# DanbiAubrey/Hypergraph_diffusion_for_recommendation

Hardware: AMD Instinct MI355X
Metric: hypergraph-conv fwd+bwd M-edges/sec at emb_dim=64; % HBM roofline (higher is better)
Workload: dtype f32

## Files before the change

hypergraph_diffusion_for_recommendation_amd/_native.py:

```python
from __future__ import annotations

import ctypes
import os
import threading

_HERE = os.path.dirname(os.path.abspath(__file__))
LIB_PATH = os.environ.get("HGD_LIB_PATH", os.path.join(_HERE, "_lib", "libhgd.so"))

c_void_p = ctypes.c_void_p
c_i64 = ctypes.c_int64
c_i32 = ctypes.c_int32
c_f32 = ctypes.c_float
c_f64 = ctypes.c_double
c_size = ctypes.c_size_t

HGD_OK = 0
EPI_NONE, EPI_LEAKY_RELU, EPI_RELU = 0, 1, 2
DT_F32, DT_BF16 = 0, 1
_STATUS_NAMES = {0: "HGD_OK", 1: "HGD_ERR_INVALID_ARG", 2: "HGD_ERR_HIP",
                 3: "HGD_ERR_UNSUPPORTED", 4: "HGD_ERR_WORKSPACE"}


class HGDNativeError(RuntimeError):
    """Raised when libhgd is missing or a call returns a non-OK hgd_status."""
# ... 195 lines not shown
                                   c_i64, c_i64, c_i64, c_void_p, c_i32, c_i64, c_void_p, c_i32,
                                   c_i64, c_i32, c_i32, c_f32, ctypes.POINTER(SplitPlan),
                                   c_void_p, c_size, c_void_p]),
    "hgd_spmm_blocks_for": (c_i32, [c_i64, c_i32]),
    "hgd_spmm_col_blocks_workspace_size": (c_size, [c_i64, c_i32]),
    "hgd_spmm_col_blocks": (c_i32, [c_void_p, c_void_p, c_i64, c_i64, c_i32, c_void_p, c_void_p,
                                    c_void_p, c_void_p, c_size, c_void_p]),
    "hgd_spmm_blocked": (c_i32, [c_void_p, c_void_p, c_void_p, c_void_p, c_i64, c_i64, c_i64,
                                 c_i64, c_void_p, c_i64, c_void_p, c_i64, c_i32, c_i32, c_f32,
                                 c_i32, c_void_p]),
    "hgd_spmm_blocked_dt_workspace_size": (c_size, [c_i64, c_i32, c_i32, c_i32]),
    "hgd_spmm_blocked_dt": (c_i32, [c_void_p, c_void_p, c_void_p, c_void_p, c_i64, c_i64, c_i64,
                                    c_i64, c_void_p, c_i32, c_i64, c_void_p, c_i32, c_i64, c_i32,
                                    c_i32, c_f32, c_i32, c_void_p, c_size, c_void_p]),
    "hgd_spmm_blocks_for_dt": (c_i32, [c_i64, c_i32, c_i32]),
    "hgd_spmm_row_order_for": (c_i32, [c_i64, c_i64, c_i64, c_i32]),
    "hgd_spmm_row_order_workspace_size": (c_size, [c_i64]),
    "hgd_spmm_row_order": (c_i32, [c_void_p, c_void_p, c_i64, c_i64, c_void_p, c_void_p,
                                   c_void_p, c_void_p, c_void_p, c_size, c_void_p]),
    "hgd_spmm_ordered": (c_i32, [c_void_p, c_void_p, c_void_p, c_void_p, c_i64, c_i64, c_i64,
                                 c_i64, c_void_p, c_i64, c_void_p, c_i64, c_i32, c_i32, c_f32,
                                 ctypes.POINTER(SplitPlan), c_void_p, c_size, c_void_p,
                                 c_void_p]),
    "hgd_spmm_masked": (c_i32, [c_void_p, c_void_p, c_void_p, c_void_p, c_f32, c_void_p, c_i64,
                                c_i64, c_i64, c_i64, c_void_p, c_i64, c_void_p, c_i64, c_i32,
                                c_i32, c_f32, ctypes.POINTER(SplitPlan), c_void_p, c_size,
                                c_void_p]),
    "hgd_spmm_masked_fused": (c_i32, [c_void_p, c_void_p, c_void_p, c_void_p, c_f32, c_void_p,
                                      c_i64, c_i64, c_i64, c_i64, c_void_p, c_i64, c_void_p,
                                      c_i64, c_i32, ctypes.POINTER(RowEpilogue),
                                      ctypes.POINTER(SplitPlan), c_void_p, c_size, c_void_p]),
    "hgd_spmm_fused": (c_i32, [c_void_p, c_void_p, c_void_p, c_void_p, c_i64, c_i64, c_i64,
                               c_i64, c_void_p, c_i64, c_void_p, c_i64, c_i32,
                               ctypes.POINTER(RowEpilogue), ctypes.POINTER(SplitPlan), c_void_p,
                               c_size, c_void_p]),
    "hgd_row_epilogue_forward": (c_i32, [c_void_p, c_i64, c_i64, c_i32,
                                         ctypes.POINTER(RowEpilogue), c_void_p, c_i64,
                                         c_void_p]),
    "hgd_row_epilogue_backward_workspace_size": (c_size, [c_i64, c_i32]),
    "hgd_row_epilogue_backward": (c_i32, [c_void_p, c_i64, c_void_p, c_i64, c_void_p, c_void_p,
                                          c_i64, c_i32, c_i32, c_f32, c_i32, c_f32, c_void_p,
                                          c_i64, c_void_p, c_void_p, c_void_p, c_size,
                                          c_void_p]),
    "hgd_linear_forward": (c_i32, [c_void_p, c_i64, c_i64, c_i32, c_void_p, c_i64, c_i32,
                                   c_void_p, c_i32, c_void_p, c_i64, c_void_p]),
    "hgd_linear_backward_data": (c_i32, [c_void_p, c_i64, c_void_p, c_i64, c_i64, c_i32,
# ... 319 lines not shown
```

hypergraph_diffusion_for_recommendation_amd/csrc/spmm.hip:

```cpp
#include <cmath>

#include <hipcub/hipcub.hpp>

#include "spmm_launch.h"

extern "C" size_t hgd_spmm_workspace_size(const hgd_split_plan* plan, int32_t d) {
  if (!plan || plan->n_heavy <= 0 || plan->threshold <= 0 || d <= 0) return 0;
  return hgd::align_up(static_cast<size_t>(plan->n_chunks) * static_cast<size_t>(d) * 4);
}

namespace hgd {
namespace {

__device__ __forceinline__ int32_t advance_block(int64_t c, int32_t k, int64_t n_cols,
                                                 int32_t n_blk) {
  while (k + 1 < n_blk && c >= n_cols * (k + 1) / n_blk) ++k;
  return k;
}

__global__ void col_block_count_kernel(const int64_t* __restrict__ rowptr,
                                       const int32_t* __restrict__ col, int64_t n_rows,
                                       int64_t n_cols, int32_t n_blk, int64_t* __restrict__ cnt) {
  const int64_t r = static_cast<int64_t>(blockIdx.x) * blockDim.x + threadIdx.x;
  if (r == 0) cnt[static_cast<int64_t>(n_blk) * n_rows] = 0;
// ... 80 lines not shown
  for (int64_t i = l; i < n; i += kOrdG) {
    col_o[dst + i] = col[src + i];
    perm[dst + i] = static_cast<int32_t>(src + i);
  }
}

struct RowOrderWs {
  size_t keys, keys_s, len, tail, total;
};

RowOrderWs row_order_ws(int64_t n_rows) {
  RowOrderWs w{};
  size_t scan = 0;
  if (hipcub::DeviceScan::ExclusiveSum(nullptr, scan, static_cast<const int64_t*>(nullptr),
                                       static_cast<int64_t*>(nullptr), n_rows + 1) != hipSuccess)
    return w;
  const size_t sort = hgd_sort_perm_workspace_size(n_rows);
  if (sort == 0) return w;
  const size_t k = align_up(static_cast<size_t>(n_rows) * sizeof(int32_t));
  w.keys = 0;
  w.keys_s = k;
  w.len = 2 * k;
  w.tail = w.len + align_up(static_cast<size_t>(n_rows + 1) * sizeof(int64_t));
  w.total = w.tail + (sort > align_up(scan) ? sort : align_up(scan));
  return w;
}

}
}

extern "C" size_t hgd_spmm_row_order_workspace_size(int64_t n_rows) {
  if (n_rows <= 0 || n_rows >= 0x7fffffffLL) return 0;
  return hgd::row_order_ws(n_rows).total;
}

extern "C" hgd_status hgd_spmm_row_order(const int64_t* rowptr, const int32_t* col,
                                         int64_t n_rows, int64_t n_cols, int32_t* order,
                                         int64_t* rowptr_o, int32_t* col_o, int32_t* perm,
                                         void* workspace, size_t workspace_bytes, void* stream) {
  using namespace hgd;
  clear_error();
  HGD_REQUIRE(n_rows >= 0 && n_cols >= 0, "hgd_spmm_row_order: negative sizes");
  HGD_REQUIRE(n_rows < 0x7fffffffLL, "hgd_spmm_row_order: n_rows >= 2^31 - 1");
  HGD_REQUIRE(n_cols < 0x7fffffffLL, "hgd_spmm_row_order: n_cols >= 2^31 - 1");
  if (n_rows == 0) return HGD_OK;
  HGD_REQUIRE(rowptr && order && rowptr_o, "hgd_spmm_row_order: null rowptr / order / rowptr_o");
// ... 16 lines not shown
  s = hgd_sort_perm(keys, n_rows, n_cols + 1, keys_s, order, ws + w.tail, workspace_bytes - w.tail,
                    stream);
  if (s != HGD_OK) return s;
  hipLaunchKernelGGL(row_order_len_kernel, dim3(grid_for(n_rows + 1)), dim3(kBlock), 0, st, rowptr,
                     order, n_rows, len);
  s = check_launch("hgd_spmm_row_order lengths");
  if (s != HGD_OK) return s;
  size_t tail_bytes = workspace_bytes - w.tail;
  HGD_HIP(hipcub::DeviceScan::ExclusiveSum(ws + w.tail, tail_bytes, len, rowptr_o, n_rows + 1, st));
  hipLaunchKernelGGL(row_order_copy_kernel, dim3(grid), dim3(kBlock), 0, st, rowptr, col, order,
                     rowptr_o, n_rows, col_o, perm);
  return check_launch("hgd_spmm_row_order copy");
}

extern "C" int32_t hgd_spmm_row_order_for(int64_t n_rows, int64_t n_src_rows, int64_t nnz,
                                          int32_t d) {
  if (n_rows <= 0 || n_src_rows <= 0 || nnz <= 0 || d <= 0) return 0;
  const double table = static_cast<double>(n_src_rows) * (d <= 128 ? d : 64) * 4.0;
  if (table < 33554432.0) return 0;
  if (nnz > 32 * n_rows) return 0;
  return 1;
}

extern "C" hgd_status hgd_spmm_ordered(const int64_t* rowptr, const int32_t* col,
                                       const float* val, const float* row_scale, int64_t n_rows,
                                       int64_t n_src_rows, int64_t row_begin, int64_t row_end,
                                       const float* X, int64_t ldx, float* Y, int64_t ldy,
                                       int32_t d, int32_t epilogue, float slope,
                                       const hgd_split_plan* plan, void* workspace,
                                       size_t workspace_bytes, const int32_t* out_row,
                                       void* stream) {
  hgd::clear_error();
  hgd::SpmmRequest r{"hgd_spmm_ordered", rowptr, col, val, row_scale, n_rows, n_src_rows, row_begin,
                     row_end, X, ldx, Y, ldy, d, epilogue, slope, plan, workspace, workspace_bytes,
                     stream};
  r.ordered = true;
  r.out_row = out_row;
  return hgd::spmm_launch<float, float>(r);
}

extern "C" hgd_status hgd_spmm(const int64_t* rowptr, const int32_t* col, const float* val,
                               const float* row_scale, int64_t n_rows, int64_t n_src_rows,
                               int64_t row_begin, int64_t row_end, const float* X, int64_t ldx,
                               float* Y, int64_t ldy, int32_t d, int32_t epilogue, float slope,
                               const hgd_split_plan* plan, void* workspace,
                               size_t workspace_bytes, void* stream) {
// ... 54 lines not shown
  if (s != HGD_OK) return s;
  HGD_HIP(hipcub::DeviceScan::ExclusiveSum(tmp, tmp_bytes, cnt, blk_start, n, st));
  hipLaunchKernelGGL(col_block_scatter_kernel, dim3(grid), dim3(256), 0, st, rowptr, col, n_rows,
                     n_cols, n_blocks, blk_start, blk_col, blk_perm);
  return check_launch("hgd_spmm_col_blocks scatter");
}

extern "C" hgd_status hgd_spmm_blocked(const int64_t* blk_start, const int32_t* blk_col,
                                       const float* blk_val, const float* row_scale,
                                       int64_t n_rows, int64_t n_src_rows, int64_t row_begin,
                                       int64_t row_end, const float* X, int64_t ldx, float* Y,
                                       int64_t ldy, int32_t d, int32_t epilogue, float slope,
                                       int32_t n_blocks, void* stream) {
  hgd::clear_error();
  hgd::SpmmRequest r{"hgd_spmm_blocked", nullptr, blk_col, blk_val, row_scale, n_rows, n_src_rows,
                     row_begin, row_end, X, ldx, Y, ldy, d, epilogue, slope};
  r.blocked = true;
  r.blk_start = blk_start;
  r.n_blk = n_blocks;
  r.stream = stream;
  return hgd::spmm_launch<float, float>(r);
}

extern "C" hgd_status hgd_spmm_fused(const int64_t* rowptr, const int32_t* col, const float* val,
                                     const float* row_scale, int64_t n_rows, int64_t n_src_rows,
                                     int64_t row_begin, int64_t row_end, const float* X,
                                     int64_t ldx, float* Y, int64_t ldy, int32_t d,
                                     const hgd_row_epilogue* epi, const hgd_split_plan* plan,
                                     void* workspace, size_t workspace_bytes, void* stream) {
  hgd::clear_error();
  HGD_REQUIRE(epi != nullptr, "hgd_spmm_fused: null epilogue descriptor");
  hgd::SpmmRequest r{"hgd_spmm_fused", rowptr, col, val, row_scale, n_rows, n_src_rows, row_begin,
                     row_end, X, ldx, Y, ldy, d, epi->act, epi->slope, plan, workspace,
                     workspace_bytes, stream};
  r.ex = epi;
  return hgd::spmm_launch<float, float>(r);
}

extern "C" hgd_status hgd_spmm_masked(const int64_t* rowptr, const int32_t* col, const float* val,
                                      const uint8_t* mask, float keep, const float* row_scale,
                                      int64_t n_rows, int64_t n_src_rows, int64_t row_begin,
                                      int64_t row_end, const float* X, int64_t ldx, float* Y,
                                      int64_t ldy, int32_t d, int32_t epilogue, float slope,
                                      const hgd_split_plan* plan, void* workspace,
                                      size_t workspace_bytes, void* stream) {
  hgd::clear_error();
// ... 30 lines not shown
```

hypergraph_diffusion_for_recommendation_amd/csrc/spmm_launch.h:

```cpp
#pragma once

#include <cmath>
#include <type_traits>

#include "spmm_kernels.h"

namespace hgd {

constexpr int kDefaultPolicy = kPolPrefetch;
static_assert(SpmmTuning{}.policy == kDefaultPolicy && SpmmTuning{}.unroll == 8);

template <class TX, class TY>
constexpr bool kF32 = std::is_same_v<TX, float> && std::is_same_v<TY, float>;

struct SpmmRequest {
  const char* fn;
  const int64_t* rowptr;
  const int32_t* col;
  const float* val;
  const float* row_scale;
  int64_t n_rows, n_src_rows;
  int64_t row_begin, row_end;
  const void* X;
  int64_t ldx;
// ... 109 lines not shown
    case 16: return launch_g<16, VEC, EX>(a, r);
    case 32: return launch_g<32, VEC, EX>(a, r);
    case 64:
      if constexpr (VEC != 8) return launch_g<64, VEC, EX>(a, r);
      [[fallthrough]];
    default: return fail(HGD_ERR_UNSUPPORTED, "%s: unsupported group size %d", r.fn, G);
  }
}

inline size_t blocked_part_bytes(int64_t n_rows, int32_t d, size_t sy, int32_t n_blk) {
  if (sy != 2 || n_blk <= 1 || n_rows <= 0 || d <= 0) return 0;
  return align_up(static_cast<size_t>(n_rows) * static_cast<size_t>(d) * 4);
}

inline bool has_split_rows(const hgd_split_plan* plan) {
  return plan && plan->threshold > 0 && plan->n_heavy > 0;
}

inline hgd_status spmm_check_args(const SpmmRequest& r) {
  const char* fn = r.fn;
  const int32_t d = r.d;
  const hgd_row_epilogue* ex = r.ex;
  const bool empty = r.row_end == r.row_begin;
  HGD_REQUIRE(!r.ordered || r.out_row || r.n_rows <= 0, "%s: null out_row", fn);
  HGD_REQUIRE(!r.blocked || (r.n_blk >= 1 && r.n_blk <= 64), "%s: blocks must be 1..64", fn);
  HGD_REQUIRE(!r.blocked || r.blk_start || r.row_end <= r.row_begin, "%s: null blk_start", fn);
  HGD_REQUIRE(r.keep > 0.f, "%s: keep must be > 0 (got %g)", fn, (double)r.keep);
  HGD_REQUIRE(!r.masked || r.mask || empty, "%s: null mask", fn);
  HGD_REQUIRE(d > 0, "%s: d must be > 0 (got %d)", fn, d);
  HGD_REQUIRE(r.n_rows >= 0 && r.n_src_rows >= 0, "%s: negative sizes", fn);
  HGD_REQUIRE(r.row_begin >= 0 && r.row_begin <= r.row_end && r.row_end <= r.n_rows,
              "%s: row range [%lld,%lld) outside [0,%lld)", fn, (long long)r.row_begin,
              (long long)r.row_end, (long long)r.n_rows);
  HGD_REQUIRE(r.ldx >= d && r.ldy >= d, "%s: ldx/ldy must be >= d", fn);
  HGD_REQUIRE(r.epilogue >= HGD_EPI_NONE && r.epilogue <= HGD_EPI_RELU, "%s: bad epilogue %d", fn,
              r.epilogue);
  if (ex) {
    HGD_REQUIRE(r.epilogue == HGD_EPI_NONE || r.slope >= 0.f,
                "%s: a fused activation needs slope >= 0 (got %g)", fn, (double)r.slope);
    HGD_REQUIRE(ex->layer_norm == 0 || ex->layer_norm == 1, "%s: layer_norm must be 0/1", fn);
    HGD_REQUIRE(!ex->res1 || ex->ld_res1 >= d, "%s: ld_res1 < d", fn);
    HGD_REQUIRE(!ex->res2 || ex->ld_res2 >= d, "%s: ld_res2 < d", fn);
    HGD_REQUIRE(!ex->act_out || ex->ld_act >= d, "%s: ld_act < d", fn);
    HGD_REQUIRE((ex->sum_out == nullptr) == (ex->sum_res == nullptr),
                "%s: sum_out and sum_res go together", fn);
    HGD_REQUIRE(!ex->sum_out || (ex->ld_sum_out >= d && ex->ld_sum_res >= d),
                "%s: ld_sum_out / ld_sum_res < d", fn);
  }
  if (!empty) {
    HGD_REQUIRE((r.rowptr || r.blocked) && r.Y, "%s: null rowptr/Y", fn);
    HGD_REQUIRE(r.X || r.n_src_rows == 0, "%s: null X", fn);
  }
  if (r.out_row) {
    if (has_split_rows(r.plan) || (r.plan && (r.plan->flags & HGD_PLAN_SEGMENTED)))
      return fail(HGD_ERR_UNSUPPORTED, "%s: no split rows or segmented walk with a row order", fn);
    if (r.mask || ex || r.blocked)
      return fail(HGD_ERR_UNSUPPORTED,
                  "%s: no mask, fused row epilogue or source blocks with a row order", fn);
    if (r.row_begin != 0 || r.row_end != r.n_rows)
      return fail(HGD_ERR_UNSUPPORTED, "%s: a row order covers all rows, got [%lld,%lld) of %lld",
                  fn, (long long)r.row_begin, (long long)r.row_end, (long long)r.n_rows);
  }
  return HGD_OK;
}

template <class TX, class TY>
hgd_status spmm_fill_args(SpmmArgsT<TX, TY>& a, const SpmmRequest& r) {
  const SpmmTuning& t = spmm_tuning();
  a.rowptr = r.rowptr;
  a.col = r.col;
  a.val = r.val;
  a.row_scale = r.row_scale;
  a.row_begin = r.row_begin;
  a.row_end = r.row_end;
  a.X = static_cast<const TX*>(r.X);
  a.ldx = r.ldx;
  a.Y = static_cast<TY*>(r.Y);
  a.ldy = r.ldy;
  a.d = r.d;
  a.epi = r.epilogue;
  a.slope = r.slope;
// ... 85 lines not shown
  return HGD_OK;
}

template <int VEC, class TX, class TY>
hgd_status spmm_passes(SpmmArgsT<TX, TY> a, const SpmmRequest& r, const SpmmPassPlan& p) {
  const int32_t d = a.d;
  const bool fused = r.ex != nullptr;
  if constexpr (kF32<TX, TY> && VEC == 4) {
    const int n_pass = (d + p.step - 1) / p.step;
    if (spmm_tuning().pass_interleave && n_pass > 1 && !fused && !r.blocked && !a.mask &&
        a.n_chunks == 0 && !a.seg) {
      a.col0 = 0;
      a.n_pass = n_pass;
      a.pass_cols = p.step;
      return launch_vec<VEC, false>(p.G, a, r);
    }
  }
  for (int c0 = 0; c0 < d; c0 += p.step) {
    a.col0 = c0;
    for (int k = 0; k < (r.blocked ? r.n_blk : 1); ++k) {
      hgd_status s;
      if (r.blocked) {
        a.rowptr = r.blk_start + static_cast<int64_t>(k) * r.n_rows;
        if constexpr (kF32<TX, TY>) {
          if (VEC == 4) a.seg = spmm_tuning().blocked_seg;
        }
        a.blk_accum = k > 0;
        a.epi = k + 1 == r.n_blk ? r.epilogue : HGD_EPI_NONE;
        a.blk_last = k + 1 == r.n_blk;
      }
      if constexpr (kF32<TX, TY>) {
        s = fused ? launch_vec<VEC, true>(p.G, a, r) : launch_vec<VEC, false>(p.G, a, r);
      } else {
        s = launch_vec<VEC, false>(p.G, a, r);
      }
      if (s != HGD_OK) return s;
    }
  }
  return HGD_OK;
}

template <class TX, class TY>
hgd_status spmm_launch(const SpmmRequest& r) {
  hgd_status s = spmm_check_args(r);
  if (s != HGD_OK || r.row_end == r.row_begin) return s;
  SpmmArgsT<TX, TY> a{};
  s = spmm_fill_args(a, r);
// ... 10 lines not shown
```

hypergraph_diffusion_for_recommendation_amd/incidence.py:

```python
from __future__ import annotations

import copy
import ctypes
import os
import weakref
from typing import Dict, Optional, Tuple

import torch

from . import _native as nat
from . import profiling

DEFAULT_SPLIT_THRESHOLD = 2048
DEFAULT_SPLIT_CHUNK = 512
SPLIT_THRESHOLD_MIN = 128
SPLIT_NNZ_PER_THRESHOLD = 8192
SEGMENTED_MAX_AVG_DEGREE = 32
TARGET_GROUPS = 16384


def auto_split(n_rows: int, nnz: int) -> Tuple[int, int]:
    if n_rows >= TARGET_GROUPS or nnz == 0:
        t = SPLIT_THRESHOLD_MIN
        while 2 * t <= nnz // SPLIT_NNZ_PER_THRESHOLD and t < DEFAULT_SPLIT_THRESHOLD:
# ... 11 lines not shown


def _stream(device) -> int:
    return nat.stream_handle(device)


class CSR:

    def __init__(self, rowptr: torch.Tensor, col: torch.Tensor, n_rows: int, n_cols: int,
                 split_threshold: int = DEFAULT_SPLIT_THRESHOLD,
                 split_chunk: int = DEFAULT_SPLIT_CHUNK, plan_counts: Optional[Tuple] = None):
        self.rowptr = rowptr
        self.col = col
        self._ws_bytes: Dict[int, int] = {}
        self.n_rows = int(n_rows)
        self.n_cols = int(n_cols)
        self.nnz = int(col.numel())
        self.device = rowptr.device
        self.split_threshold = int(split_threshold)
        self.split_chunk = int(split_chunk)
        self.cols_ascending = False
        self._col_blocks: Dict[int, Tuple[torch.Tensor, torch.Tensor, torch.Tensor]] = {}
        self._blk_vals: Dict[Tuple[int, int], tuple] = {}
        self._row_order: Optional[Tuple[torch.Tensor, ...]] = None
        self._ord_vals: Dict[Tuple[int, int], tuple] = {}
        self._plan_arrays = ()
        self.plan = nat.SplitPlan()
        self.plan.threshold = 0
        if plan_counts is not None:
            self._build_plan(*plan_counts)

    def plan_count_async(self) -> Optional[torch.Tensor]:
        if self.split_threshold <= 0 or self.n_rows == 0 or self.nnz <= self.split_threshold:
            return None
        counts = torch.empty(2, dtype=torch.int64, device=self.device)
        nat.check(nat.load().hgd_split_plan_count(
            self.rowptr.data_ptr(), self.n_rows, self.split_threshold, self.split_chunk,
            counts.data_ptr(), _stream(self.device)), "hgd_split_plan_count")
        return counts

    def _build_plan(self, n_heavy: int, n_chunks: int) -> None:
        self._ws_bytes = {}
        n_heavy, n_chunks = int(n_heavy), int(n_chunks)
        if n_heavy == 0:
            self.plan.threshold = 0
            return
# ... 41 lines not shown
                raise RuntimeError("col_blocks: the rows' columns are not known to be ascending")
            dev = self.device
            lib = nat.load()
            start = torch.empty(n_blocks * self.n_rows + 1, dtype=torch.int64, device=dev)
            bcol = torch.empty(self.nnz, dtype=torch.int32, device=dev)
            perm = torch.empty(self.nnz, dtype=torch.int32, device=dev)
            if self.n_rows:
                ws = _ws(lib.hgd_spmm_col_blocks_workspace_size(self.n_rows, n_blocks), dev)
                nat.check(lib.hgd_spmm_col_blocks(
                    self.rowptr.data_ptr(), self.col.data_ptr() if self.nnz else None,
                    self.n_rows, self.n_cols, n_blocks, start.data_ptr(),
                    bcol.data_ptr() if self.nnz else None, perm.data_ptr() if self.nnz else None,
                    ws.data_ptr(), ws.numel(), _stream(dev)), "hgd_spmm_col_blocks")
            else:
                start.zero_()
            got = self._col_blocks[n_blocks] = (start, bcol, perm)
        return got

    def blocked_values(self, n_blocks: int, val: Optional[torch.Tensor]) -> Optional[torch.Tensor]:
        if val is None:
            return None
        return _gather32_cached(self._blk_vals, n_blocks, val, self.col_blocks(n_blocks)[2])

    def row_order(self) -> Tuple[torch.Tensor, torch.Tensor, torch.Tensor, torch.Tensor]:
        got = self._row_order
        if got is None:
            dev = self.device
            lib = nat.load()
            order = torch.empty(self.n_rows, dtype=torch.int32, device=dev)
            rowptr_o = torch.empty(self.n_rows + 1, dtype=torch.int64, device=dev)
            col_o = torch.empty(self.nnz, dtype=torch.int32, device=dev)
            perm = torch.empty(self.nnz, dtype=torch.int32, device=dev)
            if self.n_rows:
                ws = _ws(lib.hgd_spmm_row_order_workspace_size(self.n_rows), dev)
                nat.check(lib.hgd_spmm_row_order(
                    self.rowptr.data_ptr(), self.col.data_ptr() if self.nnz else None,
                    self.n_rows, self.n_cols, order.data_ptr(), rowptr_o.data_ptr(),
                    col_o.data_ptr() if self.nnz else None, perm.data_ptr() if self.nnz else None,
                    ws.data_ptr(), ws.numel(), _stream(dev)), "hgd_spmm_row_order")
            else:
                rowptr_o.zero_()
            got = self._row_order = (order, rowptr_o, col_o, perm)
        return got

    def ordered_values(self, val: Optional[torch.Tensor]) -> Optional[torch.Tensor]:
        if val is None:
# ... 20 lines not shown
        return 0
    if getattr(csr, "mask", None) is not None:
        return 0
    env = os.environ.get("HGD_SPMM_BLOCKS", "")
    if env not in ("", "auto"):
        p = int(env)
        if p < 0 or p > 64:
            raise ValueError(f"HGD_SPMM_BLOCKS must be 0..64, got {env!r}")
        return p if p > 1 else 0
    return int(nat.load().hgd_spmm_blocks_for_dt(csr.n_cols, int(d), _HOP_DTYPES[x_dtype]))


def spmm_row_order(csr: CSR, d: int) -> bool:
    if csr.n_heavy or csr.segmented or csr.nnz == 0:
        return False
    if not getattr(csr, "row_order_ok", True):
        return False
    env = os.environ.get("HGD_SPMM_ROW_ORDER", "")
    if env not in ("", "auto"):
        if env not in ("0", "1"):
            raise ValueError(f"HGD_SPMM_ROW_ORDER must be 0 or 1, got {env!r}")
        return env == "1"
    return bool(nat.load().hgd_spmm_row_order_for(csr.n_rows, csr.n_cols, csr.nnz, int(d)))


_HOP_DTYPES = {torch.float32: nat.DT_F32, torch.bfloat16: nat.DT_BF16}


def spmm_csr(csr: CSR, X: torch.Tensor, val: Optional[torch.Tensor] = None,
             row_scale: Optional[torch.Tensor] = None, epilogue: int = nat.EPI_NONE,
             slope: float = 0.0, out: Optional[torch.Tensor] = None,
             row_begin: int = 0, row_end: Optional[int] = None,
             ex: Optional[nat.RowEpilogue] = None, blocks: Optional[int] = None,
             out_dtype: Optional[torch.dtype] = None) -> torch.Tensor:
    if X.dim() != 2:
        raise ValueError(f"spmm: X must be 2-D, got {tuple(X.shape)}")
    if X.dtype not in _HOP_DTYPES:
        raise TypeError(f"spmm: X must be float32 or bfloat16, got {X.dtype}")
    y_dtype = out.dtype if out is not None else (out_dtype or X.dtype)
    if y_dtype not in _HOP_DTYPES:
        raise TypeError(f"spmm: the output must be float32 or bfloat16, got {y_dtype}")
    dt = X.dtype != torch.float32 or y_dtype != torch.float32
    if dt and ex is not None:
        raise TypeError("spmm: the fused row epilogue (ex=) is float32-only; a bfloat16 "
                        f"table or output cannot take it (X {X.dtype}, output {y_dtype})")
    if X.device.type != "cuda":
# ... 15 lines not shown
        raise ValueError("spmm: row_scale size mismatch")
    lib = nat.load()
    plan_ptr = ctypes.byref(csr.plan)
    wsb = csr._ws_bytes.get(d)
    if wsb is None:
        wsb = csr._ws_bytes[d] = lib.hgd_spmm_workspace_size(plan_ptr, d)
    ws = _ws(wsb, X.device) if wsb else None
    timer = profiling.active()
    if timer is not None:
        t0 = timer.begin()
    mask = getattr(csr, "mask", None)
    if mask is not None or ex is not None or blocks == 0:
        blocks = 0
    else:
        blocks = spmm_blocks(csr, d, X.dtype)
    rp, cp, vp = csr.rowptr.data_ptr(), csr.col.data_ptr() if csr.nnz else None, nat.ptr(val)
    if mask is not None:
        mp, keep = mask.data_ptr() if csr.nnz else None, float(csr.keep)
    sp, n, m, rb, re_ = nat.ptr(row_scale), csr.n_rows, csr.n_cols, int(row_begin), int(row_end)
    xp, ldx, yp, ldy = X.data_ptr(), X.stride(0), out.data_ptr(), out.stride(0)
    wp, st = nat.ptr(ws), _stream(X.device)
    ordered = (not dt and mask is None and ex is None and not blocks and rb == 0 and re_ == n
               and spmm_row_order(csr, d))
    if ordered:
        order, rowptr_o, col_o, _ = csr.row_order()
        nat.check(lib.hgd_spmm_ordered(
            rowptr_o.data_ptr(), col_o.data_ptr(), nat.ptr(csr.ordered_values(val)),
            nat.ptr(csr.ordered_scale(row_scale)), n, m, rb, re_, xp, ldx, yp, ldy, d,
            int(epilogue), float(slope), plan_ptr, wp, wsb, order.data_ptr(), st),
            "hgd_spmm_ordered")
    elif dt and mask is not None:
        nat.check(lib.hgd_spmm_masked_dt(
            rp, cp, vp, mp, keep, sp, n, m, rb, re_, xp, _HOP_DTYPES[X.dtype], ldx, yp,
            _HOP_DTYPES[y_dtype], ldy, d, int(epilogue), float(slope), plan_ptr, wp, wsb, st),
            "hgd_spmm_masked_dt")
    elif dt and blocks:
        start, bcol, _ = csr.col_blocks(blocks)
        bval = csr.blocked_values(blocks, val)
        pb = lib.hgd_spmm_blocked_dt_workspace_size(n, d, _HOP_DTYPES[y_dtype], blocks)
        part = _ws(pb, X.device) if pb else None
        nat.check(lib.hgd_spmm_blocked_dt(
            start.data_ptr(), bcol.data_ptr(), nat.ptr(bval), sp, n, m, rb, re_, xp,
            _HOP_DTYPES[X.dtype], ldx, yp, _HOP_DTYPES[y_dtype], ldy, d, int(epilogue),
            float(slope), blocks, nat.ptr(part), pb, st), "hgd_spmm_blocked_dt")
    elif dt:
        nat.check(lib.hgd_spmm_dt(
            rp, cp, vp, sp, n, m, rb, re_, xp, _HOP_DTYPES[X.dtype], ldx, yp,
            _HOP_DTYPES[y_dtype], ldy, d, int(epilogue), float(slope), plan_ptr, wp, wsb, st),
            "hgd_spmm_dt")
    elif mask is not None and ex is not None:
        nat.check(lib.hgd_spmm_masked_fused(
            rp, cp, vp, mp, keep, sp, n, m, rb, re_, xp, ldx, yp, ldy, d, ctypes.byref(ex),
            plan_ptr, wp, wsb, st), "hgd_spmm_masked_fused")
    elif mask is not None:
        nat.check(lib.hgd_spmm_masked(
            rp, cp, vp, mp, keep, sp, n, m, rb, re_, xp, ldx, yp, ldy, d, int(epilogue),
            float(slope), plan_ptr, wp, wsb, st), "hgd_spmm_masked")
    elif ex is None and blocks:
        start, bcol, _ = csr.col_blocks(blocks)
        bval = csr.blocked_values(blocks, val)
        nat.check(lib.hgd_spmm_blocked(
            start.data_ptr(), bcol.data_ptr(), nat.ptr(bval), sp, n, m, rb, re_, xp, ldx, yp,
            ldy, d, int(epilogue), float(slope), blocks, st), "hgd_spmm_blocked")
    elif ex is None:
        nat.check(lib.hgd_spmm(
            rp, cp, vp, sp, n, m, rb, re_, xp, ldx, yp, ldy, d, int(epilogue), float(slope),
            plan_ptr, wp, wsb, st), "hgd_spmm")
    else:
        nat.check(lib.hgd_spmm_fused(
            rp, cp, vp, sp, n, m, rb, re_, xp, ldx, yp, ldy, d, ctypes.byref(ex), plan_ptr, wp,
            wsb, st), "hgd_spmm_fused")
    if timer is not None:
        full = rb == 0 and re_ == csr.n_rows

        def nbytes(csr=csr, rb=rb, re_=re_, full=full, d=d, hv=val is not None,
                   hs=row_scale is not None, blocks=blocks, xb=X.element_size(),
                   yb=out.element_size(), ordered=ordered):
            nnz = csr.nnz if full else int(csr.rowptr[re_].item() - csr.rowptr[rb].item())
            return (profiling.hop_bytes(nnz, re_ - rb, d, x_bytes=xb, y_bytes=yb),
                    profiling.impl_bytes(nnz, re_ - rb, d, hv, hs, blocks, x_bytes=xb,
                                         y_bytes=yb, ordered=ordered))

        timer.end(t0, nbytes)
    return out


class Incidence:

    def __init__(self, csr: CSR, csc: CSR, val: Optional[torch.Tensor],
                 val_t: Optional[torch.Tensor]):
        self.csr = csr
        self.csc = csc
        self.val = val
        self.val_t = val_t
        self.n_rows = csr.n_rows
        self.n_cols = csr.n_cols
        self.nnz = csr.nnz
        self.device = csr.device
        self._scales: Dict[Tuple[str, str], torch.Tensor] = {}
        self._edge_vals: Dict[Tuple[str, str, str], Optional[torch.Tensor]] = {}
        self.perm_t: Optional[torch.Tensor] = None
        self.coo_sorted = False

    @property
# ... 335 lines not shown
                                             st), "hgd_dense_threshold_rowptr")
    nnz = int(rowptr[n].item())
    cols = torch.empty(nnz, dtype=torch.int32, device=device)
    vals = torch.empty(nnz, dtype=torch.float32, device=device) if values else None
    if nnz:
        nat.check(lib.hgd_dense_threshold_fill(H.data_ptr(), n, k, H.stride(0), float(thresh),
                                               mode, rowptr.data_ptr(), cols.data_ptr(),
                                               nat.ptr(vals), st), "hgd_dense_threshold_fill")
    if values:
        return rowptr, cols, vals
    return rowptr, cols


def expand_rows(rowptr: torch.Tensor, nnz: int) -> torch.Tensor:
    n_rows = rowptr.numel() - 1
    out = torch.empty(nnz, dtype=torch.int32, device=rowptr.device)
    if nnz:
        nat.check(nat.load().hgd_expand_rows(rowptr.data_ptr(), n_rows, nnz, out.data_ptr(),
                                             _stream(rowptr.device)), "hgd_expand_rows")
    return out


def _gather32(src: torch.Tensor, perm: torch.Tensor) -> torch.Tensor:
    out = torch.empty_like(src)
    n = perm.numel()
    if n:
        nat.check(nat.load().hgd_gather32(src.data_ptr(), perm.data_ptr(), n, out.data_ptr(),
                                          _stream(src.device)), "hgd_gather32")
    return out


def _gather32_cached(cache: dict, kind: int, src: torch.Tensor,
                     perm: torch.Tensor) -> torch.Tensor:
    try:
        version = src._version
    except RuntimeError:
        return _gather32(src, perm)
    key = (kind, id(src))
    hit = cache.get(key)
    if hit is not None and hit[0]() is src and hit[1] == version:
        return hit[2]
    out = _gather32(src, perm)
    if len(cache) >= 8:
        cache.pop(next(iter(cache)))
    cache[key] = (weakref.ref(src), version, out)
    return out


# ... 22 lines not shown
```

hypergraph_diffusion_for_recommendation_amd/profiling.py:

```python
from __future__ import annotations

from typing import List, Optional

import torch

_ACTIVE: Optional["HopTimer"] = None

MODEL_NOTE = ("SURVEY.md §8d B_hop = nnz*(4+4d) + R*(4d+4) + (R+1)*4 (binary H; the folded "
              "per-nonzero source scale and the int64 rowptr are counted only in "
              "implementation_bytes_per_launch)")


def hop_bytes(nnz: int, rows: int, d: int, weighted: bool = False, x_bytes: int = 4,
              y_bytes: int = 4) -> int:
    return (nnz * (4 + (4 if weighted else 0) + x_bytes * d) + rows * (y_bytes * d + 4)
            + (rows + 1) * 4)


def impl_bytes(nnz: int, rows: int, d: int, has_val: bool, has_scale: bool,
               blocks: int = 0, x_bytes: int = 4, y_bytes: int = 4, ordered: bool = False) -> int:
    if ordered:
        return impl_bytes(nnz, rows, d, has_val, has_scale, 0, x_bytes, y_bytes) + rows * 4
    if blocks > 1:
        if y_bytes == 4:
            y_traffic = 4 * d * (2 * blocks - 1)
        else:
            y_traffic = 4 * d * (2 * blocks - 2) + y_bytes * d
        return (nnz * (4 + (4 if has_val else 0) + x_bytes * d)
                + rows * (y_traffic + (4 * blocks if has_scale else 0))
                + rows * (blocks + 1) * 8)
    return (nnz * (4 + (4 if has_val else 0) + x_bytes * d)
            + rows * (y_bytes * d + (4 if has_scale else 0)) + (rows + 1) * 8)


class HopTimer:
    def __init__(self):
        self.records: List[tuple] = []

    def __enter__(self):
        global _ACTIVE
        self._prev = _ACTIVE
        _ACTIVE = self
        return self

    def __exit__(self, *exc):
# ... 39 lines not shown
```

include/hgd.h:

```cpp
#ifndef HGD_H
#define HGD_H

#include <stddef.h>
#include <stdint.h>

#ifdef __cplusplus
extern "C" {
#endif

typedef enum hgd_status {
  HGD_OK = 0,
  HGD_ERR_INVALID_ARG = 1,
  HGD_ERR_HIP = 2,
  HGD_ERR_UNSUPPORTED = 3,
  HGD_ERR_WORKSPACE = 4
} hgd_status;

typedef enum hgd_epilogue {
  HGD_EPI_NONE = 0,
  HGD_EPI_LEAKY_RELU = 1,
  HGD_EPI_RELU = 2
} hgd_epilogue;

typedef enum hgd_tune_key {
// ... 81 lines not shown
size_t hgd_spmm_blocked_dt_workspace_size(int64_t n_rows, int32_t d, int32_t y_dtype,
                                          int32_t n_blocks);
hgd_status hgd_spmm_blocked_dt(const int64_t* blk_start, const int32_t* blk_col,
                               const float* blk_val, const float* row_scale, int64_t n_rows,
                               int64_t n_src_rows, int64_t row_begin, int64_t row_end,
                               const void* X, int32_t x_dtype, int64_t ldx, void* Y,
                               int32_t y_dtype, int64_t ldy, int32_t d, int32_t epilogue,
                               float slope, int32_t n_blocks, void* workspace,
                               size_t workspace_bytes, void* stream);
int32_t hgd_spmm_blocks_for_dt(int64_t n_src_rows, int32_t d, int32_t x_dtype);

int32_t hgd_spmm_row_order_for(int64_t n_rows, int64_t n_src_rows, int64_t nnz, int32_t d);
size_t hgd_spmm_row_order_workspace_size(int64_t n_rows);
hgd_status hgd_spmm_row_order(const int64_t* rowptr, const int32_t* col, int64_t n_rows,
                              int64_t n_cols, int32_t* order, int64_t* rowptr_o, int32_t* col_o,
                              int32_t* perm, void* workspace, size_t workspace_bytes,
                              void* stream);
hgd_status hgd_spmm_ordered(const int64_t* rowptr, const int32_t* col, const float* val,
                            const float* row_scale, int64_t n_rows, int64_t n_src_rows,
                            int64_t row_begin, int64_t row_end, const float* X, int64_t ldx,
                            float* Y, int64_t ldy, int32_t d, int32_t epilogue, float slope,
                            const hgd_split_plan* plan, void* workspace, size_t workspace_bytes,
                            const int32_t* out_row, void* stream);

hgd_status hgd_spmm_masked(const int64_t* rowptr, const int32_t* col, const float* val,
                           const uint8_t* mask, float keep, const float* row_scale,
                           int64_t n_rows, int64_t n_src_rows, int64_t row_begin,
                           int64_t row_end, const float* X, int64_t ldx, float* Y, int64_t ldy,
                           int32_t d, int32_t epilogue, float slope, const hgd_split_plan* plan,
                           void* workspace, size_t workspace_bytes, void* stream);

typedef struct hgd_row_epilogue {
  int32_t act;
  float slope;
  int32_t layer_norm;
  float ln_eps;
  const float* ln_gamma;
  const float* ln_beta;
  float out_scale;
  const float* res1;
  int64_t ld_res1;
  float res1_scale;
  const float* res2;
  int64_t ld_res2;
  float res2_scale;
  float* act_out;
// ... 456 lines not shown
```

Before: 6858.

## Add per-column-block row ordering for blocked SpMM to improve source locality

Adds a blocked-and-ordered SpMM path. Within each source-column block, rows are sorted by their minimum column key, so the gather from the feature table walks a locality-friendly order, and results are scattered back through a per-block output-row map. Preprocessing builds the sorted block CSR once and caches it, together with permuted values and row scales. The path is auto-selected only when each block's slice of the source table is large (at least 32 MiB) and the graph is not too dense. Otherwise it falls back, and it adds indirect output writes plus a one-time sort cost.

```diff
diff --git a/hypergraph_diffusion_for_recommendation_amd/_native.py b/hypergraph_diffusion_for_recommendation_amd/_native.py
--- a/hypergraph_diffusion_for_recommendation_amd/_native.py
+++ b/hypergraph_diffusion_for_recommendation_amd/_native.py
@@ -241,6 +241,14 @@
                                  c_i64, c_void_p, c_i64, c_void_p, c_i64, c_i32, c_i32, c_f32,
                                  ctypes.POINTER(SplitPlan), c_void_p, c_size, c_void_p,
                                  c_void_p]),
+    "hgd_spmm_block_order_for": (c_i32, [c_i64, c_i64, c_i64, c_i32, c_i32]),
+    "hgd_spmm_col_blocks_ordered_workspace_size": (c_size, [c_i64, c_i32]),
+    "hgd_spmm_col_blocks_ordered": (c_i32, [c_void_p, c_void_p, c_i64, c_i64, c_i32, c_void_p,
+                                            c_void_p, c_void_p, c_void_p, c_void_p, c_size,
+                                            c_void_p]),
+    "hgd_spmm_blocked_ordered": (c_i32, [c_void_p, c_void_p, c_void_p, c_void_p, c_void_p, c_i64,
+                                         c_i64, c_void_p, c_i64, c_void_p, c_i64, c_i32, c_i32,
+                                         c_f32, c_i32, c_void_p]),
     "hgd_spmm_masked": (c_i32, [c_void_p, c_void_p, c_void_p, c_void_p, c_f32, c_void_p, c_i64,
                                 c_i64, c_i64, c_i64, c_void_p, c_i64, c_void_p, c_i64, c_i32,
                                 c_i32, c_f32, ctypes.POINTER(SplitPlan), c_void_p, c_size,
diff --git a/hypergraph_diffusion_for_recommendation_amd/csrc/spmm.hip b/hypergraph_diffusion_for_recommendation_amd/csrc/spmm.hip
--- a/hypergraph_diffusion_for_recommendation_amd/csrc/spmm.hip
+++ b/hypergraph_diffusion_for_recommendation_amd/csrc/spmm.hip
@@ -126,6 +126,38 @@
   w.keys_s = k;
   w.len = 2 * k;
   w.tail = w.len + align_up(static_cast<size_t>(n_rows + 1) * sizeof(int64_t));
+  w.total = w.tail + (sort > align_up(scan) ? sort : align_up(scan));
+  return w;
+}
+
+__global__ void block_order_dest_kernel(const int64_t* __restrict__ blk_start,
+                                        const int32_t* __restrict__ out_row, int64_t n_rows,
+                                        int64_t n, int64_t* __restrict__ dest) {
+  const int64_t i = static_cast<int64_t>(blockIdx.x) * blockDim.x + threadIdx.x;
+  if (i >= n) return;
+  dest[i - i % n_rows + out_row[i]] = blk_start[i];
+}
+
+struct BlockOrderWs {
+  size_t cnt, start, keys, keys_s, tail, total;
+};
+
+BlockOrderWs block_order_ws(int64_t n_rows, int32_t n_blk) {
+  BlockOrderWs w{};
+  const int64_t n = static_cast<int64_t>(n_blk) * n_rows + 1;
+  size_t scan = 0;
+  if (hipcub::DeviceScan::ExclusiveSum(nullptr, scan, static_cast<const int64_t*>(nullptr),
+                                       static_cast<int64_t*>(nullptr), n) != hipSuccess)
+    return w;
+  const size_t sort = hgd_sort_perm_workspace_size(n_rows);
+  if (sort == 0) return w;
+  const size_t a = align_up(static_cast<size_t>(n) * sizeof(int64_t));
+  const size_t k = align_up(static_cast<size_t>(n_rows) * sizeof(int32_t));
+  w.cnt = 0;
+  w.start = a;
+  w.keys = 2 * a;
+  w.keys_s = w.keys + k;
+  w.tail = w.keys_s + k;
   w.total = w.tail + (sort > align_up(scan) ? sort : align_up(scan));
   return w;
 }
@@ -188,6 +220,16 @@
   return 1;
 }
 
+extern "C" int32_t hgd_spmm_block_order_for(int64_t n_rows, int64_t n_src_rows, int64_t nnz,
+                                            int32_t d, int32_t n_blocks) {
+  if (n_rows <= 0 || n_src_rows <= 0 || nnz <= 0 || d <= 0 || n_blocks <= 0) return 0;
+  const double slice =
+      static_cast<double>(n_src_rows) / n_blocks * (d < 128 ? d : 128) * 4.0;
+  if (slice < 33554432.0) return 0;
+  if (nnz > 32 * static_cast<int64_t>(n_blocks) * n_rows) return 0;
+  return 1;
+}
+
 extern "C" hgd_status hgd_spmm_ordered(const int64_t* rowptr, const int32_t* col,
                                        const float* val, const float* row_scale, int64_t n_rows,
                                        int64_t n_src_rows, int64_t row_begin, int64_t row_end,
@@ -288,6 +330,91 @@
   return hgd::spmm_launch<float, float>(r);
 }
 
+extern "C" size_t hgd_spmm_col_blocks_ordered_workspace_size(int64_t n_rows, int32_t n_blocks) {
+  if (n_rows <= 0 || n_rows >= 0x7fffffffLL || n_blocks <= 0 || n_blocks > 64) return 0;
+  return hgd::block_order_ws(n_rows, n_blocks).total;
+}
+
+extern "C" hgd_status hgd_spmm_col_blocks_ordered(const int64_t* rowptr, const int32_t* col,
+                                                  int64_t n_rows, int64_t n_cols,
+                                                  int32_t n_blocks, int64_t* blk_start,
+                                                  int32_t* blk_col, int32_t* blk_perm,
+                                                  int32_t* blk_out_row, void* workspace,
+                                                  size_t workspace_bytes, void* stream) {
+  using namespace hgd;
+  clear_error();
+  constexpr const char* fn = "hgd_spmm_col_blocks_ordered";
+  HGD_REQUIRE(n_rows >= 0 && n_cols >= 0, "%s: negative sizes", fn);
+  HGD_REQUIRE(n_blocks >= 1 && n_blocks <= 64, "%s: blocks must be 1..64", fn);
+  HGD_REQUIRE(n_rows < 0x7fffffffLL, "%s: n_rows >= 2^31 - 1", fn);
+  HGD_REQUIRE(n_cols < 0x7fffffffLL, "%s: n_cols >= 2^31 - 1", fn);
+  if (n_rows == 0) return HGD_OK;
+  HGD_REQUIRE(rowptr && blk_start && blk_out_row, "%s: null rowptr / blk_start / blk_out_row", fn);
+  const BlockOrderWs w = block_order_ws(n_rows, n_blocks);
+  if (w.total == 0 || !workspace || workspace_bytes < w.total)
+    return fail(HGD_ERR_WORKSPACE, "%s: workspace %zu < %zu", fn, workspace_bytes, w.total);
+  const int64_t n = static_cast<int64_t>(n_blocks) * n_rows;
+  const int64_t row_grid = (n_rows + 255) / 256;
+  constexpr int kRowsPerBlock = kBlock / kOrdG;
+  const int64_t key_grid = (n_rows + kRowsPerBlock - 1) / kRowsPerBlock;
+  hipStream_t st = as_stream(stream);
+  char* ws = static_cast<char*>(workspace);
+  int64_t* cnt = reinterpret_cast<int64_t*>(ws + w.cnt);
+  int64_t* start = reinterpret_cast<int64_t*>(ws + w.start);
+  int32_t* keys = reinterpret_cast<int32_t*>(ws + w.keys);
+  int32_t* keys_s = reinterpret_cast<int32_t*>(ws + w.keys_s);
+  size_t tail_bytes = workspace_bytes - w.tail;
+  hipLaunchKernelGGL(col_block_count_kernel, dim3(row_grid), dim3(256), 0, st, rowptr, col, n_rows,
+                     n_cols, n_blocks, cnt);
+  hgd_status s = check_launch(fn, "count");
+  if (s != HGD_OK) return s;
+  HGD_HIP(hipcub::DeviceScan::ExclusiveSum(ws + w.tail, tail_bytes, cnt, start, n + 1, st));
+  hipLaunchKernelGGL(col_block_scatter_kernel, dim3(row_grid), dim3(256), 0, st, rowptr, col,
+                     n_rows, n_cols, n_blocks, start, blk_col, static_cast<int32_t*>(nullptr));
+  s = check_launch(fn, "scatter");
+  if (s != HGD_OK) return s;
+  for (int32_t k = 0; k < n_blocks; ++k) {
+    const int64_t off = static_cast<int64_t>(k) * n_rows;
+    hipLaunchKernelGGL(row_min_key_kernel, dim3(key_grid), dim3(kBlock), 0, st, start + off,
+                       blk_col, n_rows, static_cast<int32_t>(n_cols), keys);
+    s = check_launch(fn, "keys");
+    if (s != HGD_OK) return s;
+    s = hgd_sort_perm(keys, n_rows, n_cols + 1, keys_s, blk_out_row + off, ws + w.tail, tail_bytes,
+                      stream);
+    if (s != HGD_OK) return s;
+    hipLaunchKernelGGL(row_order_len_kernel, dim3(grid_for(n_rows + 1)), dim3(kBlock), 0, st,
+                       start + off, blk_out_row + off, n_rows, cnt + off);
+    s = check_launch(fn, "lengths");
+    if (s != HGD_OK) return s;
+  }
+  HGD_HIP(hipcub::DeviceScan::ExclusiveSum(ws + w.tail, tail_bytes, cnt, blk_start, n + 1, st));
+  hipLaunchKernelGGL(block_order_dest_kernel, dim3(grid_for(n)), dim3(kBlock), 0, st, blk_start,
+                     blk_out_row, n_rows, n, start);
+  s = check_launch(fn, "destinations");
+  if (s != HGD_OK) return s;
+  hipLaunchKernelGGL(col_block_scatter_kernel, dim3(row_grid), dim3(256), 0, st, rowptr, col,
+                     n_rows, n_cols, n_blocks, start, blk_col, blk_perm);
+  return check_launch(fn, "ordered scatter");
+}
+
+extern "C" hgd_status hgd_spmm_blocked_ordered(const int64_t* blk_start, const int32_t* blk_col,
+                                               const float* blk_val, const float* blk_row_scale,
+                                               const int32_t* blk_out_row, int64_t n_rows,
+                                               int64_t n_src_rows, const float* X, int64_t ldx,
+                                               float* Y, int64_t ldy, int32_t d, int32_t epilogue,
+                                               float slope, int32_t n_blocks, void* stream) {
+  hgd::clear_error();
+  hgd::SpmmRequest r{"hgd_spmm_blocked_ordered", nullptr, blk_col, blk_val, blk_row_scale, n_rows,
+                     n_src_rows, 0, n_rows, X, ldx, Y, ldy, d, epilogue, slope};
+  r.blocked = true;
+  r.blk_start = blk_start;
+  r.n_blk = n_blocks;
+  r.ordered = true;
+  r.out_row = blk_out_row;
+  r.stream = stream;
+  return hgd::spmm_launch<float, float>(r);
+}
+
 extern "C" hgd_status hgd_spmm_fused(const int64_t* rowptr, const int32_t* col, const float* val,
                                      const float* row_scale, int64_t n_rows, int64_t n_src_rows,
                                      int64_t row_begin, int64_t row_end, const float* X,
diff --git a/hypergraph_diffusion_for_recommendation_amd/csrc/spmm_launch.h b/hypergraph_diffusion_for_recommendation_amd/csrc/spmm_launch.h
--- a/hypergraph_diffusion_for_recommendation_amd/csrc/spmm_launch.h
+++ b/hypergraph_diffusion_for_recommendation_amd/csrc/spmm_launch.h
@@ -155,7 +155,8 @@
   const int32_t d = r.d;
   const hgd_row_epilogue* ex = r.ex;
   const bool empty = r.row_end == r.row_begin;
-  HGD_REQUIRE(!r.ordered || r.out_row || r.n_rows <= 0, "%s: null out_row", fn);
+  HGD_REQUIRE(!r.ordered || r.out_row || r.n_rows <= 0, "%s: null %s", fn,
+              r.blocked ? "blk_out_row" : "out_row");
   HGD_REQUIRE(!r.blocked || (r.n_blk >= 1 && r.n_blk <= 64), "%s: blocks must be 1..64", fn);
   HGD_REQUIRE(!r.blocked || r.blk_start || r.row_end <= r.row_begin, "%s: null blk_start", fn);
   HGD_REQUIRE(r.keep > 0.f, "%s: keep must be > 0 (got %g)", fn, (double)r.keep);
@@ -187,9 +188,14 @@
   if (r.out_row) {
     if (has_split_rows(r.plan) || (r.plan && (r.plan->flags & HGD_PLAN_SEGMENTED)))
       return fail(HGD_ERR_UNSUPPORTED, "%s: no split rows or segmented walk with a row order", fn);
-    if (r.mask || ex || r.blocked)
+    if (r.blocked && r.ordered) {
+      if (r.mask || ex)
+        return fail(HGD_ERR_UNSUPPORTED, "%s: no mask or fused row epilogue with a block order",
+                    fn);
+    } else if (r.mask || ex || r.blocked) {
       return fail(HGD_ERR_UNSUPPORTED,
                   "%s: no mask, fused row epilogue or source blocks with a row order", fn);
+    }
     if (r.row_begin != 0 || r.row_end != r.n_rows)
       return fail(HGD_ERR_UNSUPPORTED, "%s: a row order covers all rows, got [%lld,%lld) of %lld",
                   fn, (long long)r.row_begin, (long long)r.row_end, (long long)r.n_rows);
@@ -321,7 +327,10 @@
       hgd_status s;
       if (r.blocked) {
         a.rowptr = r.blk_start + static_cast<int64_t>(k) * r.n_rows;
-        if constexpr (kF32<TX, TY>) {
+        if (r.ordered) {
+          a.out_row = r.out_row + static_cast<int64_t>(k) * r.n_rows;
+          if (r.row_scale) a.row_scale = r.row_scale + static_cast<int64_t>(k) * r.n_rows;
+        } else if constexpr (kF32<TX, TY>) {
           if (VEC == 4) a.seg = spmm_tuning().blocked_seg;
         }
         a.blk_accum = k > 0;
diff --git a/hypergraph_diffusion_for_recommendation_amd/incidence.py b/hypergraph_diffusion_for_recommendation_amd/incidence.py
--- a/hypergraph_diffusion_for_recommendation_amd/incidence.py
+++ b/hypergraph_diffusion_for_recommendation_amd/incidence.py
@@ -57,6 +57,8 @@
         self.cols_ascending = False
         self._col_blocks: Dict[int, Tuple[torch.Tensor, torch.Tensor, torch.Tensor]] = {}
         self._blk_vals: Dict[Tuple[int, int], tuple] = {}
+        self._col_blocks_ord: Dict[int, Tuple[torch.Tensor, ...]] = {}
+        self._blk_ord_vals: Dict[Tuple[int, int], tuple] = {}
         self._row_order: Optional[Tuple[torch.Tensor, ...]] = None
         self._ord_vals: Dict[Tuple[int, int], tuple] = {}
         self._plan_arrays = ()
@@ -144,6 +146,46 @@
             return None
         return _gather32_cached(self._blk_vals, n_blocks, val, self.col_blocks(n_blocks)[2])
 
+    def col_blocks_ordered(self, n_blocks: int) -> Tuple[torch.Tensor, ...]:
+        got = self._col_blocks_ord.get(n_blocks)
+        if got is None:
+            if not self.cols_ascending:
+                raise RuntimeError(
+                    "col_blocks_ordered: the rows' columns are not known to be ascending")
+            dev = self.device
+            lib = nat.load()
+            start = torch.empty(n_blocks * self.n_rows + 1, dtype=torch.int64, device=dev)
+            bcol = torch.empty(self.nnz, dtype=torch.int32, device=dev)
+            perm = torch.empty(self.nnz, dtype=torch.int32, device=dev)
+            out_row = torch.empty(n_blocks * self.n_rows, dtype=torch.int32, device=dev)
+            if self.n_rows:
+                ws = _ws(lib.hgd_spmm_col_blocks_ordered_workspace_size(self.n_rows, n_blocks),
+                         dev)
+                nat.check(lib.hgd_spmm_col_blocks_ordered(
+                    self.rowptr.data_ptr(), self.col.data_ptr() if self.nnz else None,
+                    self.n_rows, self.n_cols, n_blocks, start.data_ptr(),
+                    bcol.data_ptr() if self.nnz else None, perm.data_ptr() if self.nnz else None,
+                    out_row.data_ptr(), ws.data_ptr(), ws.numel(), _stream(dev)),
+                    "hgd_spmm_col_blocks_ordered")
+            else:
+                start.zero_()
+            got = self._col_blocks_ord[n_blocks] = (start, bcol, perm, out_row)
+        return got
+
+    def blocked_ordered_values(self, n_blocks: int,
+                               val: Optional[torch.Tensor]) -> Optional[torch.Tensor]:
+        if val is None:
+            return None
+        return _gather32_cached(self._blk_ord_vals, 2 * n_blocks, val,
+                                self.col_blocks_ordered(n_blocks)[2])
+
+    def blocked_ordered_scale(self, n_blocks: int,
+                              row_scale: Optional[torch.Tensor]) -> Optional[torch.Tensor]:
+        if row_scale is None:
+            return None
+        return _gather32_cached(self._blk_ord_vals, 2 * n_blocks + 1, row_scale,
+                                self.col_blocks_ordered(n_blocks)[3])
+
     def row_order(self) -> Tuple[torch.Tensor, torch.Tensor, torch.Tensor, torch.Tensor]:
         got = self._row_order
         if got is None:
@@ -210,6 +252,18 @@
             raise ValueError(f"HGD_SPMM_ROW_ORDER must be 0 or 1, got {env!r}")
         return env == "1"
     return bool(nat.load().hgd_spmm_row_order_for(csr.n_rows, csr.n_cols, csr.nnz, int(d)))
+
+
+def spmm_block_order(csr: CSR, d: int, blocks: int) -> bool:
+    if blocks <= 1 or csr.nnz == 0:
+        return False
+    env = os.environ.get("HGD_SPMM_BLOCK_ORDER", "")
+    if env not in ("", "auto"):
+        if env not in ("0", "1"):
+            raise ValueError(f"HGD_SPMM_BLOCK_ORDER must be 0 or 1, got {env!r}")
+        return env == "1"
+    return bool(nat.load().hgd_spmm_block_order_for(csr.n_rows, csr.n_cols, csr.nnz, int(d),
+                                                    int(blocks)))
 
 
 _HOP_DTYPES = {torch.float32: nat.DT_F32, torch.bfloat16: nat.DT_BF16}
@@ -271,6 +325,8 @@
     wp, st = nat.ptr(ws), _stream(X.device)
     ordered = (not dt and mask is None and ex is None and not blocks and rb == 0 and re_ == n
                and spmm_row_order(csr, d))
+    blk_ordered = (not dt and bool(blocks) and rb == 0 and re_ == n
+                   and spmm_block_order(csr, d, blocks))
     if ordered:
         order, rowptr_o, col_o, _ = csr.row_order()
         nat.check(lib.hgd_spmm_ordered(
@@ -305,6 +361,12 @@
         nat.check(lib.hgd_spmm_masked(
             rp, cp, vp, mp, keep, sp, n, m, rb, re_, xp, ldx, yp, ldy, d, int(epilogue),
             float(slope), plan_ptr, wp, wsb, st), "hgd_spmm_masked")
+    elif blk_ordered:
+        start, bcol, _, out_row = csr.col_blocks_ordered(blocks)
+        nat.check(lib.hgd_spmm_blocked_ordered(
+            start.data_ptr(), bcol.data_ptr(), nat.ptr(csr.blocked_ordered_values(blocks, val)),
+            nat.ptr(csr.blocked_ordered_scale(blocks, row_scale)), out_row.data_ptr(), n, m, xp,
+            ldx, yp, ldy, d, int(epilogue), float(slope), blocks, st), "hgd_spmm_blocked_ordered")
     elif ex is None and blocks:
         start, bcol, _ = csr.col_blocks(blocks)
         bval = csr.blocked_values(blocks, val)
@@ -324,11 +386,12 @@
 
         def nbytes(csr=csr, rb=rb, re_=re_, full=full, d=d, hv=val is not None,
                    hs=row_scale is not None, blocks=blocks, xb=X.element_size(),
-                   yb=out.element_size(), ordered=ordered):
+                   yb=out.element_size(), ordered=ordered, blk_ordered=blk_ordered):
             nnz = csr.nnz if full else int(csr.rowptr[re_].item() - csr.rowptr[rb].item())
             return (profiling.hop_bytes(nnz, re_ - rb, d, x_bytes=xb, y_bytes=yb),
                     profiling.impl_bytes(nnz, re_ - rb, d, hv, hs, blocks, x_bytes=xb,
-                                         y_bytes=yb, ordered=ordered))
+                                         y_bytes=yb, ordered=ordered,
+                                         block_ordered=blk_ordered))
 
         timer.end(t0, nbytes)
     return out
@@ -710,8 +773,8 @@
 
 
 def _gather32(src: torch.Tensor, perm: torch.Tensor) -> torch.Tensor:
-    out = torch.empty_like(src)
     n = perm.numel()
+    out = torch.empty(n, dtype=src.dtype, device=src.device)
     if n:
         nat.check(nat.load().hgd_gather32(src.data_ptr(), perm.data_ptr(), n, out.data_ptr(),
                                           _stream(src.device)), "hgd_gather32")
diff --git a/hypergraph_diffusion_for_recommendation_amd/profiling.py b/hypergraph_diffusion_for_recommendation_amd/profiling.py
--- a/hypergraph_diffusion_for_recommendation_amd/profiling.py
+++ b/hypergraph_diffusion_for_recommendation_amd/profiling.py
@@ -18,9 +18,13 @@
 
 
 def impl_bytes(nnz: int, rows: int, d: int, has_val: bool, has_scale: bool,
-               blocks: int = 0, x_bytes: int = 4, y_bytes: int = 4, ordered: bool = False) -> int:
+               blocks: int = 0, x_bytes: int = 4, y_bytes: int = 4, ordered: bool = False,
+               block_ordered: bool = False) -> int:
     if ordered:
         return impl_bytes(nnz, rows, d, has_val, has_scale, 0, x_bytes, y_bytes) + rows * 4
+    if blocks > 1 and block_ordered:
+        return (impl_bytes(nnz, rows, d, has_val, has_scale, blocks, x_bytes, y_bytes)
+                + rows * blocks * 4)
     if blocks > 1:
         if y_bytes == 4:
             y_traffic = 4 * d * (2 * blocks - 1)
diff --git a/include/hgd.h b/include/hgd.h
--- a/include/hgd.h
+++ b/include/hgd.h
@@ -127,6 +127,20 @@
                             float* Y, int64_t ldy, int32_t d, int32_t epilogue, float slope,
                             const hgd_split_plan* plan, void* workspace, size_t workspace_bytes,
                             const int32_t* out_row, void* stream);
+
+int32_t hgd_spmm_block_order_for(int64_t n_rows, int64_t n_src_rows, int64_t nnz, int32_t d,
+                                 int32_t n_blocks);
+size_t hgd_spmm_col_blocks_ordered_workspace_size(int64_t n_rows, int32_t n_blocks);
+hgd_status hgd_spmm_col_blocks_ordered(const int64_t* rowptr, const int32_t* col, int64_t n_rows,
+                                       int64_t n_cols, int32_t n_blocks, int64_t* blk_start,
+                                       int32_t* blk_col, int32_t* blk_perm, int32_t* blk_out_row,
+                                       void* workspace, size_t workspace_bytes, void* stream);
+hgd_status hgd_spmm_blocked_ordered(const int64_t* blk_start, const int32_t* blk_col,
+                                    const float* blk_val, const float* blk_row_scale,
+                                    const int32_t* blk_out_row, int64_t n_rows,
+                                    int64_t n_src_rows, const float* X, int64_t ldx, float* Y,
+                                    int64_t ldy, int32_t d, int32_t epilogue, float slope,
+                                    int32_t n_blocks, void* stream);
 
 hgd_status hgd_spmm_masked(const int64_t* rowptr, const int32_t* col, const float* val,
                            const uint8_t* mask, float keep, const float* row_scale,
```

After: 6947, median of 6. +1.3%, better.
